# nibox/Pose-Estimation-with-Message-Passing-Networks

Measured on AMD Instinct MI355X. Metric: images/sec (640px, HRNet-w48) + MPN edge-updates/sec at 1/2/4/8 MI355X, higher is better.
Workload: dtype f16x3; 1 GPU; c3: 8x17x640x640 heatmaps/GPU -> fully graph -> MPN TypeAware-attn T=3; images_per_gpu=8, global_batch=8, persons_per_image=9, nodes_per_gpu=1224, edges_per_gpu=186048, parallelism=image-sharded x1, batches_in_flight=2, detection_and_node_math=fp32

## Files before the change

include/pemp.h:

```cpp
#ifndef PEMP_H_
#define PEMP_H_

#include <stddef.h>
#include <stdint.h>

#ifdef __cplusplus
extern "C" {
#endif

#define PEMP_ABI_VERSION 24

enum {
  PEMP_OK = 0,
  PEMP_ERR_INVALID_ARG = -1,
  PEMP_ERR_HIP = -2,
  PEMP_ERR_WORKSPACE = -3,
  PEMP_ERR_UNSUPPORTED = -4,
};

int pemp_abi_version(void);
const char* pemp_last_error(void);
int pemp_device_check(void);

enum { PEMP_DETECT_NMS = 1, PEMP_DETECT_SELECT = 2, PEMP_DETECT_ALL = 3 };
// ... 168 lines not shown
  const uint16_t* upd_bf;
  const uint16_t* pre_bf;
  const float* node_img;
  const float* attn_bv;
  pemp_mlp upd_mlp;
  const float *ept_l1_w, *ept_l1_b, *ept_l2_w, *ept_l2_b, *ept_o1_w, *ept_o2_w;
  const float* edge_img;
  const uint16_t* emb_comp_bf;
  const float* emb_comp_b;
} pemp_mpn_weights;

typedef struct pemp_mpn_desc {
  int32_t num_types;
  int32_t num_joints;
  int32_t steps;
  int32_t aux_loss_steps;
  int32_t aggr;
  int32_t hidden;
  int32_t edge_attr_dim;
  int32_t node_in_dim;
  int32_t precision;
  int32_t types_stride;
  int32_t flags;
} pemp_mpn_desc;

#define PEMP_MPN_PREPARED 1
#define PEMP_MPN_TWO_LAUNCH_FIRST 4
#define PEMP_MPN_FUSED_FIRST_PROFILED 8
#define PEMP_MPN_SEPARATE_PRELUDE 16

size_t pemp_mpn_workspace_size(const pemp_mpn_desc* desc, int64_t N, int64_t E);
size_t pemp_mpn_fused_first_lds_bytes(void);
int pemp_mpn_prelude_grids(int64_t N, int64_t E, int B, int T, int nmax, int edge_grid, int cus, int32_t* out8);
int pemp_mpn_forward(const pemp_mpn_desc* desc, const pemp_mpn_weights* weights, const float* x,
                     const float* edge_attr, const int64_t* edge_index, const int64_t* node_types,
                     int64_t N, int64_t E, float* edge_logits, float* node_logits, float* class_logits,
                     void* workspace, size_t workspace_bytes, void* stream);

int pemp_mpn_forward_fully(const pemp_mpn_desc* desc, const pemp_mpn_weights* weights, const float* x,
                           const float* edge_attr, const int64_t* edge_index, const int64_t* node_types,
                           int64_t N, int64_t E, const int64_t* node_off, const int64_t* node_off_host, int B,
                           float* edge_logits, float* node_logits, float* class_logits,
                           void* workspace, size_t workspace_bytes, void* stream);

int pemp_mpn_forward_fully_cap(const pemp_mpn_desc* desc, const pemp_mpn_weights* weights, const float* x,
                               const float* edge_attr, const int64_t* node_types, int64_t n_cap, int64_t e_cap,
                               const int32_t* n_det, int det_cap, const int64_t* node_off, int B,
                               float* edge_logits, float* node_logits, float* class_logits,
                               void* workspace, size_t workspace_bytes, void* stream);

enum {
  PEMP_STEP_DET = 0, PEMP_STEP_DSC, PEMP_STEP_NDET, PEMP_STEP_X, PEMP_STEP_JDET, PEMP_STEP_JSC, PEMP_STEP_BIDX,
  PEMP_STEP_JTAGS, PEMP_STEP_EIDX, PEMP_STEP_EATTR, PEMP_STEP_NOFF, PEMP_STEP_LOGITS, PEMP_STEP_NOUT
};
typedef struct pemp_step_plan {
  int32_t B, J, H, W, pool_kernel, use_threshold, topk, det_cap, projected;
  float threshold;
  void* det_workspace;
  size_t det_workspace_bytes;
  int32_t C, F, A, mode;
  float norm_factor;
  int64_t n_cap, e_cap;
  const pemp_mpn_desc* desc;
  const pemp_mpn_weights* weights;
  void* mpn_workspace;
  size_t mpn_workspace_bytes;
// ... 132 lines not shown
```

pose-estimation-with-message-passing-networks_amd/_lib.py:

```python
import ctypes
import threading
import os

LIB_PATH = os.environ.get("PEMP_LIB") or os.path.join(os.path.dirname(os.path.abspath(__file__)), "csrc",
                                                     "libpemp.so")
ABI_VERSION = 24

ERR_INVALID_ARG, ERR_HIP, ERR_WORKSPACE, ERR_UNSUPPORTED = -1, -2, -3, -4
MPN_PREPARED, MPN_TWO_LAUNCH_FIRST, MPN_FUSED_FIRST_PROFILED = 1, 4, 8
MPN_SEPARATE_PRELUDE = 16

c_i32, c_i64, c_f32, c_sz, c_p = ctypes.c_int32, ctypes.c_int64, ctypes.c_float, ctypes.c_size_t, ctypes.c_void_p


class PempLayer(ctypes.Structure):
    _fields_ = [("w", c_p), ("b", c_p), ("in_dim", c_i32), ("out_dim", c_i32), ("relu", c_i32), ("pad_", c_i32)]


class PempMlp(ctypes.Structure):
    _fields_ = [("layer", PempLayer * 4), ("n_layers", c_i32), ("pad_", c_i32)]


class PempMpnWeights(ctypes.Structure):
    _fields_ = [("node_emb", PempMlp), ("edge_emb", PempMlp),
# ... 56 lines not shown
    "pemp_detect": (c_i32, [c_p, c_p, c_i32, c_i32, c_i32, c_i32, c_i32, c_f32, c_i32, c_i32, c_i32, c_p, c_sz,
                            c_p, c_p, c_p, c_i32, c_p, c_p]),
    "pemp_host_alloc": (c_p, [c_sz]),
    "pemp_host_free": (c_i32, [c_p]),
    "pemp_pack_nodes": (c_i32, [c_p, c_i32, c_p, c_i32, c_i32, c_i32, c_i32, c_i32, c_p, c_p, c_i32, c_p, c_i64,
                                c_p, c_p, c_p, c_p, c_p, c_p]),
    "pemp_graph_offsets": (c_i32, [c_p, c_i32, c_p, c_p, c_p]),
    "pemp_fully_graph_build": (c_i32, [c_p, c_i32, c_p, c_p, c_i32, c_p, c_i32, c_p, c_i32, c_i32, c_i32, c_i32,
                                       c_i64, c_i64, c_f32, c_i32, c_p, c_p, c_p, c_p, c_p, c_p, c_p, c_p, c_p]),
    "pemp_fully_graph_build_cap": (c_i32, [c_p, c_i32, c_p, c_p, c_i32, c_p, c_i32, c_p, c_i32, c_i32, c_i32, c_i32,
                                           c_i64, c_i64, c_f32, c_i32, c_p, c_p, c_p, c_p, c_p, c_p, c_p, c_p, c_p]),
    "pemp_fully_graph": (c_i32, [c_p, c_p, c_i32, c_i64, c_p, c_p]),
    "pemp_knn_workspace_size": (c_sz, [c_p, c_i32]),
    "pemp_knn_graph_build": (c_i32, [c_p, c_p, c_p, c_i32, c_i32, c_p, c_sz, c_i64, c_p, c_p, c_p, c_i32, c_p,
                                     c_i32, c_f32, c_i32, c_p, c_p]),
    "pemp_feature_knn_workspace_size": (c_sz, [c_p, c_i32]),
    "pemp_knn_rows_layout": (c_i32, [c_p, c_i32, c_i32, c_p]),
    "pemp_feature_knn_graph_build": (c_i32, [c_p, c_i32, c_p, c_p, c_p, c_i32, c_i32, c_p, c_sz, c_i64, c_p, c_p,
                                             c_p, c_i32, c_p, c_i32, c_f32, c_i32, c_p, c_p]),
    "pemp_score_graph_workspace_size": (c_sz, [c_p, c_i32, c_i32]),
    "pemp_score_graph": (c_i32, [c_p, c_p, c_p, c_i32, c_i32, c_i64, c_p, c_sz, c_p, c_p]),
    "pemp_gather_projected": (c_i32, [c_p, c_p, c_p, c_i32, c_i32, c_i32, c_i32, c_f32, c_p, c_p, c_i64, c_p, c_p]),
    "pemp_gather_projected_conv": (c_i32, [c_p, c_p, c_p, c_i32, c_i32, c_p, c_p, c_i32, c_i32, c_i32, c_i32, c_i32,
                                           c_f32, c_p, c_p, c_i64, c_p, c_p]),
    "pemp_detect_projected": (c_i32, [c_p, c_p, c_i32, c_i32, c_i32, c_i32, c_i32, c_f32, c_i32, c_i32, c_i32, c_p,
                                      c_sz, c_p, c_p, c_p, c_i32, c_p, c_p]),
    "pemp_gather_projected_tags": (c_i32, [c_p, c_i32, c_i32, c_i32, c_i32, c_p, c_p, c_i64, c_p, c_p]),
    "pemp_project_maps": (c_i32, [c_p, c_i32, c_i32, c_i32, c_i32, c_i32, c_p, c_p, c_p]),
    "pemp_stage_merge": (c_i32, [c_p, c_i32, c_i32, c_i32, c_p, c_i32, c_i32, c_i32, c_i32, c_i32, c_p, c_p]),
    "pemp_edge_features": (c_i32, [c_p, c_p, c_i32, c_p, c_p, c_i64, c_i32, c_f32, c_i32, c_p, c_p]),
    "pemp_mpn_workspace_size": (c_sz, [ctypes.POINTER(PempMpnDesc), c_i64, c_i64]),
    "pemp_mpn_fused_first_lds_bytes": (c_sz, []),
    "pemp_mpn_prelude_grids": (c_i32, [c_i64, c_i64, c_i32, c_i32, c_i32, c_i32, c_i32, c_p]),
    "pemp_mpn_forward": (c_i32, [ctypes.POINTER(PempMpnDesc), ctypes.POINTER(PempMpnWeights), c_p, c_p, c_p, c_p,
                                 c_i64, c_i64, c_p, c_p, c_p, c_p, c_sz, c_p]),
    "pemp_mpn_forward_fully": (c_i32, [ctypes.POINTER(PempMpnDesc), ctypes.POINTER(PempMpnWeights), c_p, c_p, c_p,
                                       c_p, c_i64, c_i64, c_p, c_p, c_i32, c_p, c_p, c_p, c_p, c_sz, c_p]),
    "pemp_mpn_forward_fully_cap": (c_i32, [ctypes.POINTER(PempMpnDesc), ctypes.POINTER(PempMpnWeights), c_p, c_p,
                                           c_p, c_i64, c_i64, c_p, c_i32, c_p, c_i32, c_p, c_p, c_p, c_p, c_sz, c_p]),
    "pemp_mpn_graph_stats": (c_i32, [c_p]),
    "pemp_edge_cus_policy": (c_i32, [c_i32, c_i64, c_i32]),
    "pemp_abi_struct_size": (c_sz, [c_i32]),
    "pemp_mpn_forward_sym": (c_i32, [ctypes.POINTER(PempMpnDesc), ctypes.POINTER(PempMpnWeights), c_p, c_p, c_p,
                                     c_p, c_i64, c_i64, c_p, c_p, c_p, c_p, c_sz, c_p]),
    "pemp_mpn_forward_knn": (c_i32, [ctypes.POINTER(PempMpnDesc), ctypes.POINTER(PempMpnWeights), c_p, c_p, c_p,
                                     c_p, c_i64, c_i64, c_p, c_p, c_p, c_p, c_p, c_i32, c_p, c_p, c_p, c_p, c_sz,
                                     c_p]),
    "pemp_mpn_prepare": (c_i32, [ctypes.POINTER(PempMpnDesc), c_p, c_p, c_i64, c_i64, c_p, c_sz, c_p]),
    "pemp_mpn_order_layout": (c_i32, [ctypes.POINTER(PempMpnDesc), c_i64, c_i64, c_p]),
    "pemp_mpn_edge_image_floats": (c_sz, [ctypes.POINTER(PempMpnDesc), ctypes.POINTER(PempMpnWeights)]),
    "pemp_mpn_edge_image": (c_i32, [ctypes.POINTER(PempMpnDesc), ctypes.POINTER(PempMpnWeights), c_p, c_sz, c_p]),
    "pemp_mpn_node_image_floats": (c_sz, [ctypes.POINTER(PempMpnWeights)]),
    "pemp_mpn_node_image": (c_i32, [ctypes.POINTER(PempMpnWeights), c_p, c_sz, c_p]),
    "pemp_mpn_status": (c_i32, [ctypes.POINTER(PempMpnDesc), c_i64, c_i64, c_p, c_p]),
    "pemp_pose_edge_weights": (c_i32, [c_p, c_i64, c_p, c_p, c_f32, c_i32, c_p, c_i32, c_i64, c_i32, c_p, c_p, c_p,
                                       c_p]),
    "pemp_pose_cluster": (c_i32, [c_i32, c_p, c_p, c_i64, c_p, c_p, c_i32, c_i32, c_p, c_p]),
    "pemp_pose_persons": (c_i32, [c_i32, c_p, c_p, c_p, c_p, c_p, c_p, c_p, c_i32, c_i32, c_i64, c_p, c_p, c_p]),
    "pemp_pose_greedy": (c_i32, [c_i32, c_p, c_p, c_i64, c_p, c_p, c_p, c_p, c_i32, c_p, c_i64, c_p, c_p]),
    "pemp_pose_fill_mean": (c_i32, [c_p, c_i32, c_i32]),
    "pemp_pose_refine_workspace_size": (c_sz, [c_i32, c_i32, c_i32, c_i32, c_i32]),
    "pemp_pose_refine": (c_i32, [c_p, c_p, c_i32, c_i32, c_i32, c_i32, c_p, c_i32, c_p, c_sz, c_p]),
    "pemp_pose_adjust": (c_i32, [c_p, c_i32, c_i32, c_i32, c_p, c_i32, c_p]),
    "pemp_pack_to_host": (c_i32, [c_i32, c_p, c_p, c_p, c_sz, c_p, c_p, c_p]),
    "pemp_pose_finish_plan": (c_i32, [c_i32, c_p, c_p, c_p, c_p, c_i32, c_p]),
    "pemp_pose_finish_batch": (c_i32, [c_p, c_p, c_i32, c_i32, c_i32, c_i32, c_i32, c_p, c_i32, c_p, c_p, c_i32,
# ... 118 lines not shown
```

pose-estimation-with-message-passing-networks_amd/csrc/mpn.hip:

```cpp
#include <limits.h>

#include <algorithm>
#include <atomic>
#include <type_traits>
#include <map>
#include <mutex>
#include <string>
#include <vector>
#include <string.h>
#include <math.h>

#include "pemp_common.h"

namespace pemp {
namespace {

constexpr int D = 64;
constexpr int LDW = 72;
constexpr int MAXT = 17;
constexpr int EDGE_WAVES = 16;
constexpr int EMB_WAVES = 16, EMB_PER_CU = 1;
constexpr int EMB_MIN_WAVES_EU = EMB_WAVES * EMB_PER_CU / 4 > 1 ? EMB_WAVES * EMB_PER_CU / 4 : 1;
constexpr int RESERVE_CUS_DEFAULT = 64;
constexpr int64_t RESERVE_MIN_EDGES = 65536;
// ... 2192 lines not shown
      off += 16 * OB * ld;
      p.src[p.n] = L.b; p.q[p.n] = 4 * OB; p.ld[p.n] = 0; p.dst[p.n] = off; p.cum[p.n] = p.total; ++p.n;
      p.total += 4 * OB;
      off += 16 * OB;
    }
  }
  return p;
}

__device__ inline void plan_element(const StagePlan& p, int idx, const float** src, int* dst) {
  const float* sp = p.src[0];
  int q = p.q[0], ld = p.ld[0], d0 = p.dst[0], cum = 0;
  for (int j = 1; j < p.n; ++j)
    if (idx >= p.cum[j]) { sp = p.src[j]; q = p.q[j]; ld = p.ld[j]; d0 = p.dst[j]; cum = p.cum[j]; }
  const int local = idx - cum, r = local / q;
  *src = sp + 4 * local;
  *dst = d0 + r * ld + 4 * (local - r * q);
}

__global__ __launch_bounds__(256) void zero_words_kernel(int* __restrict__ p, int64_t n) {
  for (int64_t i = (int64_t)blockIdx.x * blockDim.x + threadIdx.x; i < n; i += (int64_t)gridDim.x * blockDim.x) p[i] = 0;
}

__global__ __launch_bounds__(256) void stage_image_kernel(StagePlan plan, float* __restrict__ img) {
  const int64_t gid = (int64_t)blockIdx.x * blockDim.x + threadIdx.x, gs = (int64_t)gridDim.x * blockDim.x;
  for (int64_t i = gid; i < plan.total; i += gs) {
    const float* src;
    int dst;
    plan_element(plan, (int)i, &src, &dst);
    *reinterpret_cast<float4*>(img + dst) = ld4(src);
  }
}

__device__ inline void copy_to_lds(float* __restrict__ lds, const float* __restrict__ src, int n) {
  const int n4 = n >> 2, bs = blockDim.x;
  for (int base = threadIdx.x; base < n4; base += 8 * bs) {
    float4 t[8];
#pragma unroll
    for (int k = 0; k < 8; ++k) t[k] = ld4(src + 4 * min(base + k * bs, n4 - 1));
    __builtin_amdgcn_sched_barrier(0);
#pragma unroll
    for (int k = 0; k < 8; ++k)
      if (base + k * bs < n4) *reinterpret_cast<float4*>(&lds[4 * (base + k * bs)]) = t[k];
  }
}

__device__ inline void dma_to_lds(float* __restrict__ lds, const float* __restrict__ src, int n) {
  const int lane = threadIdx.x & 63, wave = threadIdx.x >> 6, nw = blockDim.x >> 6;
  const int pieces = n >> 8, tail = n - (pieces << 8);
  for (int k = wave; k < pieces; k += nw) dma16(src + 256 * k + 4 * lane, lds + 256 * k);
  if (tail && wave == nw - 1 && 4 * lane < tail)
    *reinterpret_cast<float4*>(&lds[256 * pieces + 4 * lane]) = ld4(src + 256 * pieces + 4 * lane);
}
__device__ __forceinline__ void lds_drain() { asm volatile("s_waitcnt vmcnt(0)" ::: "memory"); }

__device__ inline void mlp_lds_frag(const float* lds, const pemp_mlp& m, float (&a)[4][4]) {
  float b[4][4];
  int off = 0;
  for (int l = 0; l < m.n_layers; ++l) {
    const pemp_layer& L = m.layer[l];
    const int KB = (L.in_dim + 15) >> 4, OB = (L.out_dim + 15) >> 4, ld = lds_stride(16 * KB);
    layer_lds(lds + off, ld, lds + off + 16 * OB * ld, KB, OB, L.relu, a, b);
    off += 16 * OB * ld + 16 * OB;
#pragma unroll
    for (int x = 0; x < 4; ++x)
#pragma unroll
      for (int r = 0; r < 4; ++r) a[x][r] = b[x][r];
  }
}

enum { ROWS_NONE = 0, ROWS_EMBED = 1, ROWS_SUM = 2, ROWS_COPY = 3 };

struct NodeRowsArgs {
  int mode;
  const float* x_in;
  int in_ld;
  pemp_mlp emb;
  const float* agg;
  const int* seg;
  int T;
  const float* upd_b;
  int64_t N;
  float* X;
  pemp_mlp node_head, class_head;
  int J;
  float *node_out, *node_out2, *class_out, *class_out2;
  const float* img;
  int head_off, head_floats;
  const int64_t* ne;
  int slot, dup;
  int emb_whole;
};

static int max_layer_floats(const pemp_mlp& m) {
  int mx = 0;
  for (int l = 0; l < m.n_layers; ++l) {
    const int KB = (m.layer[l].in_dim + 15) >> 4, OB = (m.layer[l].out_dim + 15) >> 4;
    mx = std::max(mx, 16 * OB * lds_stride(16 * KB) + 16 * OB);
  }
  return mx;
}

constexpr int NODE_ROWS_LDS_MAX = 160 * 1024;

static bool node_emb_whole(const pemp_mlp& emb) {
  return (size_t)(3 * 16 * RS + mlp_lds_floats(emb)) * sizeof(float) <= (size_t)NODE_ROWS_LDS_MAX;
}

static size_t node_rows_lds_bytes(const NodeRowsArgs& a) {
  int region = 0;
  if (a.mode == ROWS_EMBED) region = a.emb_whole ? mlp_lds_floats(a.emb) : max_layer_floats(a.emb);
  if (a.node_out) region = std::max(region, a.head_floats);
  return (size_t)(3 * 16 * RS + region) * sizeof(float);
}

__device__ __forceinline__ void node_rows_role(const NodeRowsArgs& a, float* lds, int bx) {
  float* xs = lds;
  float* act0 = lds + 16 * RS;
  float* act1 = act0 + 16 * RS;
  float* wreg = act1 + 16 * RS;
  const int lane = threadIdx.x & 63, wave = threadIdx.x >> 6, c = lane & 15, g = lane >> 4;
  const int64_t n0 = (int64_t)bx * 16, N = a.ne ? a.ne[0] : a.N;
  if (n0 >= N) return;
  const bool heads = a.node_out != nullptr;
  float *node_out = a.node_out, *node_out2 = a.node_out2, *class_out = a.class_out, *class_out2 = a.class_out2;
  if (a.ne && heads) {
    node_out = a.node_out + (int64_t)a.slot * N;
    class_out = a.class_out + (int64_t)a.slot * N * a.J;
    node_out2 = a.dup ? node_out + N : nullptr;
    class_out2 = a.dup ? class_out + N * a.J : nullptr;
  }
  const int r = threadIdx.x >> 4, q = threadIdx.x & 15;
  const int64_t n = n0 + r, nc = n < N ? n : N - 1;
  if (a.mode == ROWS_EMBED) {
    const bool whole = a.emb_whole != 0;
    if (whole) dma_to_lds(wreg, a.img, mlp_lds_floats(a.emb));
    const int K0 = a.emb.layer[0].in_dim, KP = (K0 + 15) & ~15;
    for (int base = threadIdx.x; base < 16 * KP; base += 8 * 256) {
      float v[8];
#pragma unroll
      for (int k = 0; k < 8; ++k) {
        const int idx = base + 256 * k, rr = idx / KP, kk = idx - rr * KP;
        v[k] = (idx < 16 * KP && kk < K0) ? a.x_in[min(n0 + rr, N - 1) * a.in_ld + kk] : 0.0f;
      }
#pragma unroll
      for (int k = 0; k < 8; ++k) {
        const int idx = base + 256 * k, rr = idx / KP, kk = idx - rr * KP;
        if (idx < 16 * KP) act0[rr * RS + kk] = v[k];
      }
    }
    int cur = 0, off = 0;
    for (int l = 0; l < a.emb.n_layers; ++l) {
      const pemp_layer& L = a.emb.layer[l];
      const int KB = (L.in_dim + 15) >> 4, OB = (L.out_dim + 15) >> 4, ld = lds_stride(16 * KB);
      const int lf = 16 * OB * ld + 16 * OB;
      if (whole) {
        if (l == 0) lds_drain();
      } else {
        if (l > 0) __syncthreads();
        copy_to_lds(wreg, a.img + off, lf);
      }
      __syncthreads();
      const float* Wl = whole ? wreg + off : wreg;
      off += lf;
      const float* bl = Wl + 16 * OB * ld;
      const float* src = cur ? act1 : act0;
      float* dst = cur ? act0 : act1;
      for (int ob = wave; ob < OB; ob += 4) {
        const float4 bb = ld4(bl + 16 * ob + 4 * g);
        f32x4 acc = {bb.x, bb.y, bb.z, bb.w};
        for (int mb = 0; mb < KB; ++mb) {
          const float4 w = ld4(Wl + (16 * ob + c) * ld + 16 * mb + 4 * g);
          const float4 xv = ld4(&src[c * RS + 16 * mb + 4 * g]);
          acc = mfma4(w.x, xv.x, acc);
          acc = mfma4(w.y, xv.y, acc);
          acc = mfma4(w.z, xv.z, acc);
          acc = mfma4(w.w, xv.w, acc);
        }
        if (L.relu) {
#pragma unroll
          for (int k = 0; k < 4; ++k) acc[k] = fmaxf(acc[k], 0.0f);
        }
        st4(&dst[c * RS + 16 * ob + 4 * g], acc[0], acc[1], acc[2], acc[3]);
      }
      cur ^= 1;
    }
    __syncthreads();
    if (heads) dma_to_lds(wreg, a.img + a.head_off, a.head_floats);
    const float* res = cur ? act1 : act0;
    const float4 v = ld4(&res[r * RS + 4 * q]);
    *reinterpret_cast<float4*>(&xs[r * RS + 64 + 4 * q]) = v;
    if (n < N) {
      *reinterpret_cast<float4*>(a.X + n * 128 + 4 * q) = v;
      *reinterpret_cast<float4*>(a.X + n * 128 + 64 + 4 * q) = v;
    }
  } else {
    if (heads) dma_to_lds(wreg, a.img + a.head_off, a.head_floats);
    float4 v;
    if (a.mode == ROWS_SUM) {
      float4 y[MAXT];
      int s0[MAXT], s1[MAXT];
      const int T = a.T;
#pragma unroll
      for (int t = 0; t < MAXT; ++t) {
        const int tc = min(t, T - 1);
        y[t] = ld4(a.agg + (nc * T + tc) * D + 4 * q);
        s0[t] = a.seg[tc * N + nc];
        s1[t] = a.seg[tc * N + nc + 1];
      }
      v = ld4(a.upd_b + 4 * q);
#pragma unroll
      for (int t = 0; t < MAXT; ++t) {
        if (t < T && s1[t] > s0[t]) { v.x += y[t].x; v.y += y[t].y; v.z += y[t].z; v.w += y[t].w; }
      }
      v = make_float4(fmaxf(v.x, 0.f), fmaxf(v.y, 0.f), fmaxf(v.z, 0.f), fmaxf(v.w, 0.f));
    } else if (a.mode == ROWS_COPY) {
      const float4 y = ld4(a.agg + nc * D + 4 * q);
      v = a.seg[nc + 1] > a.seg[nc] ? y : make_float4(0.f, 0.f, 0.f, 0.f);
    } else {
      v = ld4(a.X + nc * 128 + 64 + 4 * q);
    }
    *reinterpret_cast<float4*>(&xs[r * RS + 64 + 4 * q]) = v;
    if (a.mode != ROWS_NONE && n < N) *reinterpret_cast<float4*>(a.X + n * 128 + 64 + 4 * q) = v;
  }
  if (!heads) return;
  lds_drain();
  __syncthreads();
  if (wave < 2) {
    float in[4][4];
#pragma unroll
    for (int mb = 0; mb < 4; ++mb) {
      const float4 x = ld4(&xs[c * RS + 64 + 16 * mb + 4 * g]);
      in[mb][0] = x.x; in[mb][1] = x.y; in[mb][2] = x.z; in[mb][3] = x.w;
    }
    const pemp_mlp& m = wave == 0 ? a.node_head : a.class_head;
    mlp_lds_frag(wave == 0 ? wreg : wreg + mlp_lds_floats(a.node_head), m, in);
    const int od = wave == 0 ? 1 : a.J;
    float* o1 = wave == 0 ? node_out : class_out;
    float* o2 = wave == 0 ? node_out2 : class_out2;
    const int64_t nn = n0 + c;
    if (nn < N) {
#pragma unroll
      for (int ob = 0; ob < 4; ++ob)
#pragma unroll
        for (int k = 0; k < 4; ++k) {
          const int f = 16 * ob + 4 * g + k;
          if (f < od) {
            o1[nn * od + f] = in[ob][k];
            if (o2) o2[nn * od + f] = in[ob][k];
          }
        }
    }
  }
}

__global__ __launch_bounds__(256) void node_rows_kernel(NodeRowsArgs a) {
  extern __shared__ __attribute__((aligned(16))) float lds[];
  node_rows_role(a, lds, blockIdx.x);
}

struct NodeTableArgs {
  const float* X;
  int64_t N;
  const float *pre_w, *pre_b;
  const uint16_t* pre_bf;
  int NO, groups;
  float* NT;
  const int64_t* ne;
  const float* agg;
  const int* seg;
  int T;
  const float* upd_b;
};

constexpr int64_t NODE_SUM_TABLE_MAX_MB = 16;
constexpr int TBL_TILES = 2;

template <int PREC, int TILES, bool SUM>
__device__ __forceinline__ void node_table_role(const NodeTableArgs& a, float* xs, int bx) {
  static_assert(!SUM || TILES == 1, "the summing variant takes one 16-node tile per workgroup");
  const int lane = threadIdx.x & 63, wave = threadIdx.x >> 6, c = lane & 15, g = lane >> 4;
  const int chunk = bx / a.groups, grp = bx - chunk * a.groups;
  const int64_t n0 = (int64_t)chunk * 16 * TILES, N = a.ne ? a.ne[0] : a.N;
  if (n0 >= N) return;
  const int nob = a.NO / 16, ob = grp * 4 + wave, obc = min(ob, nob - 1);
  float4 w[8];
  bf16x8_t wh[4], wlo[4];
  f16x8_t fh[4], flo[4];
  if (PREC == 0) {
#pragma unroll
    for (int mb = 0; mb < 8; ++mb) w[mb] = ld4(a.pre_w + (int64_t)(16 * obc + c) * 128 + 16 * mb + 4 * g);
// ... 364 lines not shown
    const int before = lo - s0;
    const int64_t d = ob + dl;
    const int pos = tbase[t] + (int)cb_sh[t] + dl * (s1 - s0) - before;
    const bool d_in = lty[dl] == t;
    if (part == 0) a.seg[(int64_t)t * N + d] = pos;
    for (int m = s0 + part; m < s1; m += FULLY_PARTS) {
      const int i = sorted[m];
      if (i == dl) continue;
      const int p = pos + (m - s0) - (d_in && i > dl ? 1 : 0);
      a.s_src[p] = ob + i;
      a.s_dst[p] = (int)d;
      a.s_orig[p] = (int)(eoff + (long long)i * (nb - 1) + (dl < i ? dl : dl - 1));
    }
  }
  if (bx == 0 && by == 0) {
    if (threadIdx.x == 0) {
      a.seg[(int64_t)T * N] = tbase[T];
      a.err[0] = bad_sh ? 2 : 0;
      a.err[1] = a.err[2] = a.err[3] = 0;
    }
    type_split(tbase, tbase[T], T, a.Gsplit, gt_sh, a.wg_start);
  }
}

__global__ __launch_bounds__(256) void fully_prepare_kernel(FullyPrepArgs a) {
  __shared__ FullyPrepLds s;
  fully_prepare_role(a, s, blockIdx.x, blockIdx.y, gridDim.x);
}

__global__ __launch_bounds__(256) void prelude_a_kernel(FullyPrepArgs fa, NodeRowsArgs na, int split, int gx) {
  extern __shared__ __attribute__((aligned(16))) float lds[];
  const int bx = blockIdx.x;
  if (bx < split) fully_prepare_role(fa, *reinterpret_cast<FullyPrepLds*>(lds), bx % gx, bx / gx, gx);
  else node_rows_role(na, lds, bx - split);
}

static size_t prelude_a_lds_bytes(const NodeRowsArgs& na) {
  return std::max(node_rows_lds_bytes(na), sizeof(FullyPrepLds));
}

constexpr int SYM_TBITS = 24;
constexpr unsigned SYM_NMASK = (1u << SYM_TBITS) - 1u;

__device__ int64_t wave_lower_bound(const int64_t* __restrict__ a, int64_t n, int64_t key) {
  const int lane = threadIdx.x & 63;
  int64_t lo = 0, hi = n;
  while (lo < hi) {
    const int64_t s = (hi - lo + 63) / 64;
    const int64_t q = lo + (int64_t)lane * s;
    const unsigned long long m = __ballot(q < hi && a[q] < key);
    const int c = __popcll(m);
    if (c == 0) break;
    const int64_t nlo = lo + (int64_t)(c - 1) * s + 1, nhi = min(hi, lo + (int64_t)c * s);
    lo = nlo;
    hi = nhi;
  }
  return lo;
}

__global__ __launch_bounds__(256) void sym_rows_kernel(const int64_t* __restrict__ ei, const int64_t* __restrict__ types,
                                                       int64_t ts, int64_t N, int64_t E, int T, int* __restrict__ cnt,
                                                       int2* __restrict__ rows, unsigned* __restrict__ packed,
                                                       int* __restrict__ flags) {
  const int lane = threadIdx.x & 63;
  const int64_t n = (int64_t)blockIdx.x * 4 + (threadIdx.x >> 6);
  if (n >= N) return;
  const int64_t r0 = wave_lower_bound(ei, E, n);
  int f = 0, tcount = 0;
  int64_t r = r0, prev = -1;
  for (;;) {
    const int64_t e = r + lane;
    const bool in = e < E && ei[e] == n;
// ... 779 lines not shown
    } else {
      hipLaunchKernelGGL(edge_embed_wide_kernel, dim3((unsigned)((E + 63) / 64)), dim3(256), 0, st, w.edge_emb,
                         c.edge_attr, d.edge_attr_dim, ws.s_orig, E, w.q0_w, w.q0_b, w.e1_w, ws.EA, ws.Q0,
                         d.precision == PEMP_PREC_F16X3 ? dom<2>() : 1.0f);
    }
    PEMP_LAUNCH_CHECK();
    return PEMP_OK;
  }

  NodeRowsArgs rows_args(int mode, int slot, bool dup) const {
    const pemp_mpn_weights& w = *c.w;
    const int64_t N = c.N;
    const int J = p.J;
    NodeRowsArgs na{};
    na.mode = mode;
    if (mode == ROWS_EMBED) { na.x_in = c.x; na.in_ld = c.desc->node_in_dim; }
    na.agg = ws.agg; na.seg = ws.seg; na.T = p.T; na.upd_b = w.upd_b; na.N = N; na.X = ws.X;
    na.node_head = w.node_head; na.class_head = w.class_head; na.J = J;
    na.ne = ne;
    if (slot >= 0 && p.fused_heads && ne) {
      na.node_out = c.node_logits;
      na.class_out = c.class_logits;
      na.slot = slot;
      na.dup = dup ? 1 : 0;
    } else if (slot >= 0 && p.fused_heads) {
      na.node_out = c.node_logits + (int64_t)slot * N;
      na.class_out = c.class_logits + (int64_t)slot * N * J;
      na.node_out2 = dup ? na.node_out + N : nullptr;
      na.class_out2 = dup ? na.class_out + N * J : nullptr;
    }
    na.emb = w.node_emb;
    na.img = node_img;
    na.head_off = p.fused_embed ? mlp_lds_floats(w.node_emb) : 0;
    na.head_floats = mlp_lds_floats(w.node_head) + mlp_lds_floats(w.class_head);
    na.emb_whole = mode == ROWS_EMBED && node_emb_whole(w.node_emb);
    return na;
  }

  NodeTableArgs table_args() const {
    return NodeTableArgs{ws.X, c.N, c.w->pre_w, c.w->pre_b, c.w->pre_bf, p.NO, p.table_groups, ws.NT, ne};
  }

  int launch_paired() {
    const PreludeGrids& g = p.grids;
    const FullyPrepArgs fa = fully_args();
    const NodeRowsArgs na = rows_args(ROWS_EMBED, -1, false);
    hipLaunchKernelGGL(prelude_a_kernel, dim3((unsigned)(g.a_split + g.rows_blocks)), dim3(256),
                       prelude_a_lds_bytes(na), st, fa, na, g.a_split, g.a_gx);
    PEMP_LAUNCH_CHECK();
    const EdgeRangesArgs ra = ranges_args();
    const NodeTableArgs ta = table_args();
    with_prec(p.table_prec, [&](auto P) {
      hipLaunchKernelGGL(prelude_b_kernel<decltype(P)::value>, dim3((unsigned)(g.b_split + g.table_blocks)), dim3(256),
                         0, st, ra, ta, g.b_split);
    });
    PEMP_LAUNCH_CHECK();
    return PEMP_OK;
  }

  int node_step(int mode, bool table, int slot, bool dup) {
    const pemp_mpn_weights& w = *c.w;
    const int64_t N = c.N;
    const int T = p.T, J = p.J;
    if (mode == ROWS_SUM && table && slot < 0 && p.sum_in_table) {
      NodeTableArgs ta{ws.X, N, w.pre_w, w.pre_b, w.pre_bf, p.NO, p.table_groups, ws.NT, ne, ws.agg, ws.seg, T,
                       w.upd_b};
      ProfScope prof("node_update_table", st);
      with_prec(p.table_prec, [&](auto P) {
        hipLaunchKernelGGL((node_table_kernel<decltype(P)::value, 1, true>), dim3(p.table_grid1), dim3(256), 0, st, ta);
      });
      PEMP_LAUNCH_CHECK();
      return PEMP_OK;
    }
    if (mode == NODE_UPDATE_MLP && w.upd_mlp.n_layers > 0) {
      NodeMlpArgs ma{ws.agg, ws.seg, T, N, w.upd_mlp, nmlp_max_out(w.upd_mlp), ws.X, ne};
      ProfScope prof("node_update", st);
      hipLaunchKernelGGL(node_mlp_kernel, dim3(p.node_grid), dim3(256), nmlp_lds_bytes(T, w.upd_mlp), st, ma);
      PEMP_LAUNCH_CHECK();
      mode = ROWS_NONE;
    } else if (mode == NODE_UPDATE_MLP) {
      NodeUpdateArgs ua{ws.agg, ws.seg, T, N, w.upd_w, w.upd_b, ws.X, ne};
      ProfScope prof("node_update", st);
      hipLaunchKernelGGL(node_update_kernel, dim3(p.node_grid, 4), dim3(64 * UPD_WAVES), 0, st, ua);
      PEMP_LAUNCH_CHECK();
      mode = ROWS_NONE;
    }
    const NodeRowsArgs na = rows_args(mode, slot, dup);
    if (na.mode != ROWS_NONE || na.node_out) {
      ProfScope prof(mode == ROWS_EMBED ? "node_embed" : "node_update", st);
      hipLaunchKernelGGL(node_rows_kernel, dim3(p.node_grid), dim3(256), node_rows_lds_bytes(na), st, na);
      PEMP_LAUNCH_CHECK();
    }
    if (slot >= 0 && !p.fused_heads) {
      for (int k = 0; k < (dup ? 2 : 1); ++k) {
        int r2;
        if ((r2 = rows_mlp("heads", w.node_head, ws.X + 64, 128, N, c.node_logits + (int64_t)(slot + k) * N, 1, nullptr,
                           0, st)))
          return r2;
        if ((r2 = rows_mlp("heads", w.class_head, ws.X + 64, 128, N, c.class_logits + (int64_t)(slot + k) * N * J, J,
                           nullptr, 0, st)))
          return r2;
      }
    }
    if (table) {
      const NodeTableArgs ta = table_args();
      ProfScope prof("node_table", st);
      with_prec(p.table_prec, [&](auto P) {
        hipLaunchKernelGGL(node_table_kernel<decltype(P)::value>, dim3(p.table_grid), dim3(256), 0, st, ta);
      });
      PEMP_LAUNCH_CHECK();
      return launch_ept();
    }
    return PEMP_OK;
  }

  int launch_ept() {
    if (!p.ept) return PEMP_OK;
    const pemp_mpn_weights& w = *c.w;
    NodeEptArgs xa{ws.X, c.node_types, p.tstride, p.T, c.N, w.ept_l1_w, w.ept_l1_b, w.ept_l2_w, w.ept_l2_b,
                   w.ept_o1_w, w.ept_o2_w, ws.NT, p.NO,
                   c.desc->precision == PEMP_PREC_F16X3 ? dom<2>() : 1.0f, ne};
    hipLaunchKernelGGL(node_ept_kernel, dim3(p.node_grid), dim3(256), 0, st, xa);
    PEMP_LAUNCH_CHECK();
// ... 339 lines not shown
                 "pemp_mpn_prepare: N=%lld E=%lld out of range", (long long)N, (long long)E);
  PEMP_CHECK_ARG(E == 0 || (edge_index && node_types), "pemp_mpn_prepare: null edge tensors");
  size_t need = 0;
  mpn_carve(nullptr, desc->num_types, N, E, &need);
  if (workspace_bytes < need) {
    set_error("pemp_mpn_prepare: workspace %zu < %zu bytes", workspace_bytes, need);
    return PEMP_ERR_WORKSPACE;
  }
  if (N == 0) return PEMP_OK;
  return launch_prepare(desc, edge_index, node_types, N, E, mpn_carve(workspace, desc->num_types, N, E, nullptr),
                        as_stream(stream));
}

extern "C" int pemp_mpn_order_layout(const pemp_mpn_desc* desc, int64_t N, int64_t E, size_t* offs) {
  PEMP_CHECK_ARG(desc && offs && desc->num_types >= 1 && desc->num_types <= MAXT, "pemp_mpn_order_layout: bad desc");
  PEMP_CHECK_ARG(N >= 0 && E >= 0, "pemp_mpn_order_layout: N=%lld E=%lld out of range", (long long)N, (long long)E);
  mpn_carve(nullptr, desc->num_types, N, E, nullptr, offs);
  return PEMP_OK;
}

extern "C" size_t pemp_mpn_fused_first_lds_bytes(void) { return edge_first_lds_bytes(); }

extern "C" int pemp_mpn_prelude_grids(int64_t N, int64_t E, int B, int T, int nmax, int edge_grid, int cus,
                                      int32_t* out8) {
  PEMP_CHECK_ARG(out8 && N >= 0 && E >= 0 && B >= 0 && B <= FULLY_MAXB && T >= 1 && T <= MAXT && nmax >= 0 &&
                     nmax <= FULLY_MAXN && edge_grid >= 1 && cus >= 1,
                 "pemp_mpn_prelude_grids: bad args");
  const PreludeGrids g = prelude_grids(N, E, B, T, nmax, edge_grid, cus);
  static_assert(sizeof(PreludeGrids) == 8 * sizeof(int32_t), "eight ints");
  memcpy(out8, &g, sizeof(g));
  return PEMP_OK;
}

extern "C" size_t pemp_mpn_edge_image_floats(const pemp_mpn_desc* desc, const pemp_mpn_weights* w) {
  if (!desc || !w || desc->num_types < 1 || desc->num_types > MAXT) return 0;
  if (!mlp_ok(w->edge_emb, 64, 64)) return edge_image_base_floats(*desc, *w);
  return embed_image_offset(*desc, *w) + embed_image_floats(embed_layout(w->edge_emb, embed_prec(*desc, *w)));
}

extern "C" int pemp_mpn_edge_image(const pemp_mpn_desc* desc, const pemp_mpn_weights* w, float* image, size_t floats,
                                   void* stream) {
  PEMP_CHECK_ARG(desc && w && image, "pemp_mpn_edge_image: null pointer");
  PEMP_CHECK_ARG(desc->num_types >= 1 && desc->num_types <= MAXT, "pemp_mpn_edge_image: bad num_types");
  PEMP_CHECK_ARG(desc->precision == PEMP_PREC_FP32 || (w->e1_bf && w->e2_bf && w->msg_bf),
                 "pemp_mpn_edge_image: split precisions need the *_bf packs");
  PEMP_CHECK_ARG(w->e1_w && w->e2_w && w->e2_b && w->msg_w, "pemp_mpn_edge_image: null layer weights");
  PEMP_CHECK_ARG(desc->aggr != PEMP_AGGR_ATTN || w->attn_w, "pemp_mpn_edge_image: attention needs attn_w");
  const size_t need = pemp_mpn_edge_image_floats(desc, w);
  PEMP_CHECK_ARG(floats >= need, "pemp_mpn_edge_image: image needs %zu floats", need);
  EdgeImgArgs ia = edge_image_args(*desc, *w, edge_upd_fused(*desc, *w), edge_pub_head(*desc, *w), image);
  hipLaunchKernelGGL(edge_image_kernel, dim3(16, (unsigned)desc->num_types), dim3(256), 0, as_stream(stream), ia);
  PEMP_LAUNCH_CHECK();
  if (mlp_ok(w->edge_emb, 64, 64)) {
    const int prec = embed_prec(*desc, *w);
    const EmbedLayout lo = embed_layout(w->edge_emb, prec);
    float* eimg = image + embed_image_offset(*desc, *w);
    const bool fixed = embed_fixed_shape(lo);
    const bool comp = embed_composed(lo, prec, *w);
    with_prec(prec, [&](auto P) {
      constexpr int PREC = decltype(P)::value;
      auto launch = [&](auto FX) {
        hipLaunchKernelGGL((embed_image_kernel<PREC, decltype(FX)::value>), dim3(16), dim3(256), 0, as_stream(stream),
                           w->edge_emb, lo, w->emb_bf, w->q0_w, w->q0_b, w->e1_w, w->e1_bf,
                           comp ? w->emb_comp_bf : nullptr, comp ? w->emb_comp_b : nullptr, eimg);
      };
      if constexpr (PREC != PEMP_PREC_FP32)
// ... 42 lines not shown
```

Baseline: 35920 images/s.

## Keep node-row MLP weights in registers instead of staging them through LDS

The node embedding and head MLPs in node_rows no longer copy weight images into LDS. Each wave loads its output-block weight fragments straight from global memory into registers and prefetches the next layer's fragments while computing the current one. This shrinks the kernel's dynamic LDS to the activation buffers, which should allow more blocks per CU and removes the copy and drain stalls. The costs are higher register pressure, repeated global weight loads per block, and a fixed 8-K-block cap on embedding input width. The prelude kernel also gets a compile-time embed-only specialization and a fixed LDS size.

Measured after the change: 36450 images/s (median of 6 runs). 1.01x the previous value.

```diff
diff --git a/include/pemp.h b/include/pemp.h
--- a/include/pemp.h
+++ b/include/pemp.h
@@ -224,6 +224,7 @@
 size_t pemp_mpn_workspace_size(const pemp_mpn_desc* desc, int64_t N, int64_t E);
 size_t pemp_mpn_fused_first_lds_bytes(void);
 int pemp_mpn_prelude_grids(int64_t N, int64_t E, int B, int T, int nmax, int edge_grid, int cus, int32_t* out8);
+size_t pemp_mpn_node_rows_lds_bytes(const pemp_mpn_desc* desc, int mode, int heads);
 int pemp_mpn_forward(const pemp_mpn_desc* desc, const pemp_mpn_weights* weights, const float* x,
                      const float* edge_attr, const int64_t* edge_index, const int64_t* node_types,
                      int64_t N, int64_t E, float* edge_logits, float* node_logits, float* class_logits,
diff --git a/pose-estimation-with-message-passing-networks_amd/_lib.py b/pose-estimation-with-message-passing-networks_amd/_lib.py
--- a/pose-estimation-with-message-passing-networks_amd/_lib.py
+++ b/pose-estimation-with-message-passing-networks_amd/_lib.py
@@ -112,6 +112,7 @@
     "pemp_mpn_workspace_size": (c_sz, [ctypes.POINTER(PempMpnDesc), c_i64, c_i64]),
     "pemp_mpn_fused_first_lds_bytes": (c_sz, []),
     "pemp_mpn_prelude_grids": (c_i32, [c_i64, c_i64, c_i32, c_i32, c_i32, c_i32, c_i32, c_p]),
+    "pemp_mpn_node_rows_lds_bytes": (c_sz, [ctypes.POINTER(PempMpnDesc), c_i32, c_i32]),
     "pemp_mpn_forward": (c_i32, [ctypes.POINTER(PempMpnDesc), ctypes.POINTER(PempMpnWeights), c_p, c_p, c_p, c_p,
                                  c_i64, c_i64, c_p, c_p, c_p, c_p, c_sz, c_p]),
     "pemp_mpn_forward_fully": (c_i32, [ctypes.POINTER(PempMpnDesc), ctypes.POINTER(PempMpnWeights), c_p, c_p, c_p,
diff --git a/pose-estimation-with-message-passing-networks_amd/csrc/mpn.hip b/pose-estimation-with-message-passing-networks_amd/csrc/mpn.hip
--- a/pose-estimation-with-message-passing-networks_amd/csrc/mpn.hip
+++ b/pose-estimation-with-message-passing-networks_amd/csrc/mpn.hip
@@ -2248,19 +2248,6 @@
   }
 }
 
-__device__ inline void copy_to_lds(float* __restrict__ lds, const float* __restrict__ src, int n) {
-  const int n4 = n >> 2, bs = blockDim.x;
-  for (int base = threadIdx.x; base < n4; base += 8 * bs) {
-    float4 t[8];
-#pragma unroll
-    for (int k = 0; k < 8; ++k) t[k] = ld4(src + 4 * min(base + k * bs, n4 - 1));
-    __builtin_amdgcn_sched_barrier(0);
-#pragma unroll
-    for (int k = 0; k < 8; ++k)
-      if (base + k * bs < n4) *reinterpret_cast<float4*>(&lds[4 * (base + k * bs)]) = t[k];
-  }
-}
-
 __device__ inline void dma_to_lds(float* __restrict__ lds, const float* __restrict__ src, int n) {
   const int lane = threadIdx.x & 63, wave = threadIdx.x >> 6, nw = blockDim.x >> 6;
   const int pieces = n >> 8, tail = n - (pieces << 8);
@@ -2270,19 +2257,85 @@
 }
 __device__ __forceinline__ void lds_drain() { asm volatile("s_waitcnt vmcnt(0)" ::: "memory"); }
 
-__device__ inline void mlp_lds_frag(const float* lds, const pemp_mlp& m, float (&a)[4][4]) {
-  float b[4][4];
-  int off = 0;
-  for (int l = 0; l < m.n_layers; ++l) {
-    const pemp_layer& L = m.layer[l];
-    const int KB = (L.in_dim + 15) >> 4, OB = (L.out_dim + 15) >> 4, ld = lds_stride(16 * KB);
-    layer_lds(lds + off, ld, lds + off + 16 * OB * ld, KB, OB, L.relu, a, b);
-    off += 16 * OB * ld + 16 * OB;
-#pragma unroll
-    for (int x = 0; x < 4; ++x)
-#pragma unroll
-      for (int r = 0; r < 4; ++r) a[x][r] = b[x][r];
-  }
+struct ImgLayer {
+  const float *w, *b;
+  int KB, OB, ld, relu;
+};
+
+__device__ __forceinline__ ImgLayer img_layer(const float* at, const pemp_layer& L) {
+  ImgLayer G;
+  G.KB = (L.in_dim + 15) >> 4;
+  G.OB = (L.out_dim + 15) >> 4;
+  G.ld = lds_stride(16 * G.KB);
+  G.relu = L.relu;
+  G.w = at;
+  G.b = at + 16 * G.OB * G.ld;
+  return G;
+}
+
+__device__ __forceinline__ const float* img_layer_end(const ImgLayer& G) { return G.b + 16 * G.OB; }
+
+template <int NB>
+__device__ __forceinline__ void load_wfrag(const ImgLayer& G, int ob, int c, int g, float4 (&w)[NB], float4& b) {
+  const int obc = min(ob, G.OB - 1);
+  const float* row = G.w + (16 * obc + c) * G.ld + 4 * g;
+#pragma unroll
+  for (int mb = 0; mb < NB; ++mb) w[mb] = ld4(row + 16 * min(mb, G.KB - 1));
+  b = ld4(G.b + 16 * obc + 4 * g);
+}
+
+struct HeadFrags {
+  float4 w[4][4], b[4];
+  ImgLayer G;
+};
+
+__device__ __forceinline__ void head_frags_first(HeadFrags& h, const float* at, const pemp_mlp& m, int c, int g) {
+  h.G = img_layer(at, m.layer[0]);
+#pragma unroll
+  for (int ob = 0; ob < 4; ++ob) load_wfrag<4>(h.G, ob, c, g, h.w[ob], h.b[ob]);
+}
+
+template <bool AHEAD>
+__device__ __forceinline__ void head_frags_layer(HeadFrags& h, const ImgLayer& Gn, int c, int g, float (&a)[4][4]) {
+  float out[4][4];
+#pragma unroll
+  for (int ob = 0; ob < 4; ++ob) {
+    if (ob < h.G.OB) {
+      f32x4 acc = {h.b[ob].x, h.b[ob].y, h.b[ob].z, h.b[ob].w};
+#pragma unroll
+      for (int mb = 0; mb < 4; ++mb) {
+        if (mb < h.G.KB) {
+          const float4 w = h.w[ob][mb];
+          acc = mfma4(w.x, a[mb][0], acc);
+          acc = mfma4(w.y, a[mb][1], acc);
+          acc = mfma4(w.z, a[mb][2], acc);
+          acc = mfma4(w.w, a[mb][3], acc);
+        }
+      }
+#pragma unroll
+      for (int r = 0; r < 4; ++r) out[ob][r] = h.G.relu ? relu1(acc[r]) : acc[r];
+    } else {
+#pragma unroll
+      for (int r = 0; r < 4; ++r) out[ob][r] = 0.0f;
+    }
+    if (AHEAD) {
+      __builtin_amdgcn_sched_barrier(0);
+      load_wfrag<4>(Gn, ob, c, g, h.w[ob], h.b[ob]);
+    }
+  }
+#pragma unroll
+  for (int x = 0; x < 4; ++x)
+#pragma unroll
+    for (int r = 0; r < 4; ++r) a[x][r] = out[x][r];
+}
+
+__device__ __forceinline__ void head_frags_run(HeadFrags& h, const pemp_mlp& m, int c, int g, float (&a)[4][4]) {
+  for (int l = 1; l < m.n_layers; ++l) {
+    const ImgLayer Gn = img_layer(img_layer_end(h.G), m.layer[l]);
+    head_frags_layer<true>(h, Gn, c, g, a);
+    h.G = Gn;
+  }
+  head_frags_layer<false>(h, h.G, c, g, a);
 }
 
 enum { ROWS_NONE = 0, ROWS_EMBED = 1, ROWS_SUM = 2, ROWS_COPY = 3 };
@@ -2302,43 +2355,59 @@
   int J;
   float *node_out, *node_out2, *class_out, *class_out2;
   const float* img;
-  int head_off, head_floats;
+  int head_off;
   const int64_t* ne;
   int slot, dup;
-  int emb_whole;
 };
 
-static int max_layer_floats(const pemp_mlp& m) {
-  int mx = 0;
-  for (int l = 0; l < m.n_layers; ++l) {
-    const int KB = (m.layer[l].in_dim + 15) >> 4, OB = (m.layer[l].out_dim + 15) >> 4;
-    mx = std::max(mx, 16 * OB * lds_stride(16 * KB) + 16 * OB);
-  }
-  return mx;
-}
-
-constexpr int NODE_ROWS_LDS_MAX = 160 * 1024;
-
-static bool node_emb_whole(const pemp_mlp& emb) {
-  return (size_t)(3 * 16 * RS + mlp_lds_floats(emb)) * sizeof(float) <= (size_t)NODE_ROWS_LDS_MAX;
-}
-
-static size_t node_rows_lds_bytes(const NodeRowsArgs& a) {
-  int region = 0;
-  if (a.mode == ROWS_EMBED) region = a.emb_whole ? mlp_lds_floats(a.emb) : max_layer_floats(a.emb);
-  if (a.node_out) region = std::max(region, a.head_floats);
-  return (size_t)(3 * 16 * RS + region) * sizeof(float);
-}
-
+static size_t node_rows_lds_bytes() { return (size_t)(3 * 16 * RS) * sizeof(float); }
+
+__device__ __forceinline__ void embed_out_block(const ImgLayer& G, int ob, int c, int g, const float4 (&w)[8],
+                                                const float4& b, const float* src, float* dst) {
+  if (ob >= G.OB) return;
+  f32x4 acc = {b.x, b.y, b.z, b.w};
+#pragma unroll
+  for (int mb = 0; mb < 8; ++mb) {
+    if (mb < G.KB) {
+      const float4 xv = ld4(&src[c * RS + 16 * mb + 4 * g]);
+      acc = mfma4(w[mb].x, xv.x, acc);
+      acc = mfma4(w[mb].y, xv.y, acc);
+      acc = mfma4(w[mb].z, xv.z, acc);
+      acc = mfma4(w[mb].w, xv.w, acc);
+    }
+  }
+  if (G.relu) {
+#pragma unroll
+    for (int k = 0; k < 4; ++k) acc[k] = fmaxf(acc[k], 0.0f);
+  }
+  st4(&dst[c * RS + 16 * ob + 4 * g], acc[0], acc[1], acc[2], acc[3]);
+}
+
+__device__ __forceinline__ void lds_barrier() { asm volatile("s_waitcnt lgkmcnt(0)\n\ts_barrier" ::: "memory"); }
+
+template <bool AHEAD>
+__device__ __forceinline__ void embed_layer(const ImgLayer& G, const ImgLayer& Gn, int wave, int c, int g,
+                                            float4 (&wa)[8], float4& ba, float4 (&wb)[8], float4& bb,
+                                            const float* src, float* dst) {
+  lds_barrier();
+  embed_out_block(G, wave, c, g, wa, ba, src, dst);
+  if (AHEAD) load_wfrag<8>(Gn, wave, c, g, wa, ba);
+  embed_out_block(G, wave + 4, c, g, wb, bb, src, dst);
+  if (AHEAD && Gn.OB > 4) load_wfrag<8>(Gn, wave + 4, c, g, wb, bb);
+}
+
+template <bool EMBED_ONLY>
 __device__ __forceinline__ void node_rows_role(const NodeRowsArgs& a, float* lds, int bx) {
   float* xs = lds;
   float* act0 = lds + 16 * RS;
   float* act1 = act0 + 16 * RS;
-  float* wreg = act1 + 16 * RS;
-  const int lane = threadIdx.x & 63, wave = threadIdx.x >> 6, c = lane & 15, g = lane >> 4;
+  const int lane = threadIdx.x & 63, c = lane & 15, g = lane >> 4;
+  const int wave = __builtin_amdgcn_readfirstlane(threadIdx.x >> 6);
   const int64_t n0 = (int64_t)bx * 16, N = a.ne ? a.ne[0] : a.N;
   if (n0 >= N) return;
-  const bool heads = a.node_out != nullptr;
+  const bool heads = !EMBED_ONLY && a.node_out != nullptr;
+  const float* head_img = a.img + a.head_off + (wave == 0 ? 0 : mlp_lds_floats(a.node_head));
+  HeadFrags hf;
   float *node_out = a.node_out, *node_out2 = a.node_out2, *class_out = a.class_out, *class_out2 = a.class_out2;
   if (a.ne && heads) {
     node_out = a.node_out + (int64_t)a.slot * N;
@@ -2348,9 +2417,12 @@
   }
   const int r = threadIdx.x >> 4, q = threadIdx.x & 15;
   const int64_t n = n0 + r, nc = n < N ? n : N - 1;
-  if (a.mode == ROWS_EMBED) {
-    const bool whole = a.emb_whole != 0;
-    if (whole) dma_to_lds(wreg, a.img, mlp_lds_floats(a.emb));
+  if (EMBED_ONLY || a.mode == ROWS_EMBED) {
+    const int nl = a.emb.n_layers;
+    ImgLayer G = img_layer(a.img, a.emb.layer[0]);
+    float4 wa[8], wb[8], ba, bb;
+    load_wfrag<8>(G, wave, c, g, wa, ba);
+    load_wfrag<8>(G, wave + 4, c, g, wb, bb);
     const int K0 = a.emb.layer[0].in_dim, KP = (K0 + 15) & ~15;
     for (int base = threadIdx.x; base < 16 * KP; base += 8 * 256) {
       float v[8];
@@ -2365,44 +2437,17 @@
         if (idx < 16 * KP) act0[rr * RS + kk] = v[k];
       }
     }
-    int cur = 0, off = 0;
-    for (int l = 0; l < a.emb.n_layers; ++l) {
-      const pemp_layer& L = a.emb.layer[l];
-      const int KB = (L.in_dim + 15) >> 4, OB = (L.out_dim + 15) >> 4, ld = lds_stride(16 * KB);
-      const int lf = 16 * OB * ld + 16 * OB;
-      if (whole) {
-        if (l == 0) lds_drain();
-      } else {
-        if (l > 0) __syncthreads();
-        copy_to_lds(wreg, a.img + off, lf);
-      }
-      __syncthreads();
-      const float* Wl = whole ? wreg + off : wreg;
-      off += lf;
-      const float* bl = Wl + 16 * OB * ld;
-      const float* src = cur ? act1 : act0;
-      float* dst = cur ? act0 : act1;
-      for (int ob = wave; ob < OB; ob += 4) {
-        const float4 bb = ld4(bl + 16 * ob + 4 * g);
-        f32x4 acc = {bb.x, bb.y, bb.z, bb.w};
-        for (int mb = 0; mb < KB; ++mb) {
-          const float4 w = ld4(Wl + (16 * ob + c) * ld + 16 * mb + 4 * g);
-          const float4 xv = ld4(&src[c * RS + 16 * mb + 4 * g]);
-          acc = mfma4(w.x, xv.x, acc);
-          acc = mfma4(w.y, xv.y, acc);
-          acc = mfma4(w.z, xv.z, acc);
-          acc = mfma4(w.w, xv.w, acc);
-        }
-        if (L.relu) {
-#pragma unroll
-          for (int k = 0; k < 4; ++k) acc[k] = fmaxf(acc[k], 0.0f);
-        }
-        st4(&dst[c * RS + 16 * ob + 4 * g], acc[0], acc[1], acc[2], acc[3]);
-      }
+    int cur = 0;
+    for (int l = 1; l < nl; ++l) {
+      const ImgLayer Gn = img_layer(img_layer_end(G), a.emb.layer[l]);
+      embed_layer<true>(G, Gn, wave, c, g, wa, ba, wb, bb, cur ? act1 : act0, cur ? act0 : act1);
+      G = Gn;
       cur ^= 1;
     }
+    embed_layer<false>(G, G, wave, c, g, wa, ba, wb, bb, cur ? act1 : act0, cur ? act0 : act1);
+    cur ^= 1;
     __syncthreads();
-    if (heads) dma_to_lds(wreg, a.img + a.head_off, a.head_floats);
+    if (heads && wave < 2) head_frags_first(hf, head_img, wave == 0 ? a.node_head : a.class_head, c, g);
     const float* res = cur ? act1 : act0;
     const float4 v = ld4(&res[r * RS + 4 * q]);
     *reinterpret_cast<float4*>(&xs[r * RS + 64 + 4 * q]) = v;
@@ -2410,8 +2455,8 @@
       *reinterpret_cast<float4*>(a.X + n * 128 + 4 * q) = v;
       *reinterpret_cast<float4*>(a.X + n * 128 + 64 + 4 * q) = v;
     }
-  } else {
-    if (heads) dma_to_lds(wreg, a.img + a.head_off, a.head_floats);
+  } else if (!EMBED_ONLY) {
+    const bool first = heads && wave < 2;
     float4 v;
     if (a.mode == ROWS_SUM) {
       float4 y[MAXT];
@@ -2430,17 +2475,21 @@
         if (t < T && s1[t] > s0[t]) { v.x += y[t].x; v.y += y[t].y; v.z += y[t].z; v.w += y[t].w; }
       }
       v = make_float4(fmaxf(v.x, 0.f), fmaxf(v.y, 0.f), fmaxf(v.z, 0.f), fmaxf(v.w, 0.f));
-    } else if (a.mode == ROWS_COPY) {
-      const float4 y = ld4(a.agg + nc * D + 4 * q);
-      v = a.seg[nc + 1] > a.seg[nc] ? y : make_float4(0.f, 0.f, 0.f, 0.f);
+      __builtin_amdgcn_sched_barrier(0);
+      if (first) head_frags_first(hf, head_img, wave == 0 ? a.node_head : a.class_head, c, g);
     } else {
-      v = ld4(a.X + nc * 128 + 64 + 4 * q);
+      if (first) head_frags_first(hf, head_img, wave == 0 ? a.node_head : a.class_head, c, g);
+      if (a.mode == ROWS_COPY) {
+        const float4 y = ld4(a.agg + nc * D + 4 * q);
+        v = a.seg[nc + 1] > a.seg[nc] ? y : make_float4(0.f, 0.f, 0.f, 0.f);
+      } else {
+        v = ld4(a.X + nc * 128 + 64 + 4 * q);
+      }
     }
     *reinterpret_cast<float4*>(&xs[r * RS + 64 + 4 * q]) = v;
     if (a.mode != ROWS_NONE && n < N) *reinterpret_cast<float4*>(a.X + n * 128 + 64 + 4 * q) = v;
   }
   if (!heads) return;
-  lds_drain();
   __syncthreads();
   if (wave < 2) {
     float in[4][4];
@@ -2450,7 +2499,7 @@
       in[mb][0] = x.x; in[mb][1] = x.y; in[mb][2] = x.z; in[mb][3] = x.w;
     }
     const pemp_mlp& m = wave == 0 ? a.node_head : a.class_head;
-    mlp_lds_frag(wave == 0 ? wreg : wreg + mlp_lds_floats(a.node_head), m, in);
+    head_frags_run(hf, m, c, g, in);
     const int od = wave == 0 ? 1 : a.J;
     float* o1 = wave == 0 ? node_out : class_out;
     float* o2 = wave == 0 ? node_out2 : class_out2;
@@ -2472,7 +2521,7 @@
 
 __global__ __launch_bounds__(256) void node_rows_kernel(NodeRowsArgs a) {
   extern __shared__ __attribute__((aligned(16))) float lds[];
-  node_rows_role(a, lds, blockIdx.x);
+  node_rows_role<false>(a, lds, blockIdx.x);
 }
 
 struct NodeTableArgs {
@@ -2903,12 +2952,12 @@
   extern __shared__ __attribute__((aligned(16))) float lds[];
   const int bx = blockIdx.x;
   if (bx < split) fully_prepare_role(fa, *reinterpret_cast<FullyPrepLds*>(lds), bx % gx, bx / gx, gx);
-  else node_rows_role(na, lds, bx - split);
-}
-
-static size_t prelude_a_lds_bytes(const NodeRowsArgs& na) {
-  return std::max(node_rows_lds_bytes(na), sizeof(FullyPrepLds));
-}
+  else node_rows_role<true>(na, lds, bx - split);
+}
+
+constexpr size_t PRELUDE_A_LDS = 96 * 1024;
+static_assert(PRELUDE_A_LDS >= sizeof(FullyPrepLds), "launch A's LDS holds the order's arrays");
+static size_t prelude_a_lds_bytes() { return std::max(node_rows_lds_bytes(), PRELUDE_A_LDS); }
 
 constexpr int SYM_TBITS = 24;
 constexpr unsigned SYM_NMASK = (1u << SYM_TBITS) - 1u;
@@ -3754,8 +3803,6 @@
     na.emb = w.node_emb;
     na.img = node_img;
     na.head_off = p.fused_embed ? mlp_lds_floats(w.node_emb) : 0;
-    na.head_floats = mlp_lds_floats(w.node_head) + mlp_lds_floats(w.class_head);
-    na.emb_whole = mode == ROWS_EMBED && node_emb_whole(w.node_emb);
     return na;
   }
 
@@ -3768,7 +3815,7 @@
     const FullyPrepArgs fa = fully_args();
     const NodeRowsArgs na = rows_args(ROWS_EMBED, -1, false);
     hipLaunchKernelGGL(prelude_a_kernel, dim3((unsigned)(g.a_split + g.rows_blocks)), dim3(256),
-                       prelude_a_lds_bytes(na), st, fa, na, g.a_split, g.a_gx);
+                       prelude_a_lds_bytes(), st, fa, na, g.a_split, g.a_gx);
     PEMP_LAUNCH_CHECK();
     const EdgeRangesArgs ra = ranges_args();
     const NodeTableArgs ta = table_args();
@@ -3810,7 +3857,7 @@
     const NodeRowsArgs na = rows_args(mode, slot, dup);
     if (na.mode != ROWS_NONE || na.node_out) {
       ProfScope prof(mode == ROWS_EMBED ? "node_embed" : "node_update", st);
-      hipLaunchKernelGGL(node_rows_kernel, dim3(p.node_grid), dim3(256), node_rows_lds_bytes(na), st, na);
+      hipLaunchKernelGGL(node_rows_kernel, dim3(p.node_grid), dim3(256), node_rows_lds_bytes(), st, na);
       PEMP_LAUNCH_CHECK();
     }
     if (slot >= 0 && !p.fused_heads) {
@@ -4216,6 +4263,12 @@
   return PEMP_OK;
 }
 
+extern "C" size_t pemp_mpn_node_rows_lds_bytes(const pemp_mpn_desc* desc, int mode, int heads) {
+  if (!desc || mode < ROWS_NONE || mode > ROWS_COPY) return 0;
+  (void)heads;
+  return node_rows_lds_bytes();
+}
+
 extern "C" size_t pemp_mpn_edge_image_floats(const pemp_mpn_desc* desc, const pemp_mpn_weights* w) {
   if (!desc || !w || desc->num_types < 1 || desc->num_types > MAXT) return 0;
   if (!mlp_ok(w->edge_emb, 64, 64)) return edge_image_base_floats(*desc, *w);
```
